# Stanford-ILIAD/PantheonRL

Measured on AMD Instinct MI355X. Metric: env-steps/sec (all agents) Overcooked-simple PPO self-play, higher is better.
Workload: dtype f32; 1 GPU; OvercookedMultiEnv-v0 layout=simple, PPO self-play (two independent PPO learners per GPU), synthetic (n_envs, n_steps, obs_dim) rollouts; n_envs=1024, n_steps=128, obs_dim=62, features=62, n_logits=6, batch_size=32768, n_epochs=10, agents_per_gpu=2, parallelism=2 agent(s) per gpu x1 gpu(s) = 2 learners (single process), launch_mode=graph, gemm_mode=2, action_masks=none, rollout=scripted, rollout_requested=scripted

## Files before the change

### pantheonrl_amd/csrc/ph_policy.hip

```cpp
#include <cstring>
#include <initializer_list>
#include "ph_rowtail.h"
#include "ph_liar_group.h"
#include "ph_pool.h"

namespace ph {


template <int R, int LP, bool VALU>
__device__ __forceinline__ void policy_fwd_body(const FwdArgs& a) {
  extern __shared__ __attribute__((aligned(16))) float smem[];
  constexpr int NT = R * 4;
  const NetDims& nd = a.nd;
  constexpr int Lp = LP, LDO = LP + 1;
  float* bufA = smem;
  float* bufB = bufA + R * LDH;
  float* w1s = bufB + R * LDH;
  float* w2s = w1s + HID * LDH;
  float* wos = w2s + HID * LDH;
  float* outs = wos + HID * LDO;
  float* b1s = outs + R * LDO;
  float* b2s = b1s + HID;
  float* bos = b2s + HID;
  int* rowphys = (int*)(bos + 64);

  const int tid = threadIdx.x;
  const int wave = tid >> 6, lane = tid & 63, li = lane & 31, lh = lane >> 5;
  const int mt = wave >> 1, nt = wave & 1;
  const int net = blockIdx.y;
  const int row0 = blockIdx.x * R;
  const ph_layout& lay = nd.lay;
  const float* W1 = a.params + (net == 0 ? lay.pi_W1 : lay.vf_W1);
  const float* B1 = a.params + (net == 0 ? lay.pi_b1 : lay.vf_b1);
  const float* W2 = a.params + (net == 0 ? lay.pi_W2 : lay.vf_W2);
  const float* B2 = a.params + (net == 0 ? lay.pi_b2 : lay.vf_b2);

  PH_STAMP(a.prof, 0);
  if (tid < R) rowphys[tid] = (row0 + tid < a.n) ? row0 + tid : -1;
  WStage<NT> w2r, w1r;
  WoStage<NT> wor;
  XStage<R, NT> xr;
  w2r.issue(W2, 0, HID);
  w1r.issue(W1, 0, nd.F);
  if (net == 0) wor.issue(a.params + lay.act_W, nd.L, Lp);
  float bias1 = 0.f, bias2 = 0.f, bias3 = 0.f;
  if (tid < HID) {
    bias1 = B1[tid];
    bias2 = B2[tid];
    bias3 = (net == 0) ? ((tid < nd.L) ? a.params[lay.act_b + tid] : 0.f) : a.params[lay.val_W + tid];
  }
  PH_STAMP(a.prof, 8);
  __syncthreads();
  PH_STAMP(a.prof, 9);
  xr.issue(rowphys, a.obs, nd, 0);
  w2r.commit(w2s);
  PH_STAMP(a.prof, 10);
  w1r.commit(w1s);
  if (net == 0) wor.commit(wos, Lp, LDO);
  if (tid < HID) {
    b1s[tid] = bias1;
    b2s[tid] = bias2;
    bos[tid] = bias3;
  }
  PH_STAMP(a.prof, 11);
  xr.commit(bufA, rowphys, a.obs, nd, 0);
  __syncthreads();
  PH_STAMP(a.prof, 1);

  f32x16 acc = {0};
  for (int c = 0; c < nd.nchunk; ++c) {
    if (c > 0) {
      __syncthreads();
      w1r.issue(W1, c * HID, nd.F);
      xr.issue(rowphys, a.obs, nd, c);
      w1r.commit(w1s);
      xr.commit(bufA, rowphys, a.obs, nd, c);
      __syncthreads();
    }
    PH_STAMP(a.prof, 2);
    acc = tile_mma<false, false, VALU>(bufA, LDH, w1s, LDH, mt * 32, nt * 32, 0, HID, acc);
  }
  PH_STAMP(a.prof, 3);
#pragma unroll
  for (int r = 0; r < 16; ++r) {
    const int row = mt * 32 + drow(r, lh), col = nt * 32 + li;
    bufB[row * LDH + col] = fast_tanh(acc[r] + b1s[col]);
  }
  __syncthreads();
  PH_STAMP(a.prof, 4);

  f32x16 acc2 = {0};
  acc2 = tile_mma<false, false, VALU>(bufB, LDH, w2s, LDH, mt * 32, nt * 32, 0, HID, acc2);
#pragma unroll
  for (int r = 0; r < 16; ++r) {
    const int row = mt * 32 + drow(r, lh), col = nt * 32 + li;
    bufA[row * LDH + col] = fast_tanh(acc2[r] + b2s[col]);
  }
  __syncthreads();
  PH_STAMP(a.prof, 5);

  if (net == 1) {
    if (tid < R && rowphys[tid] >= 0) {
      float v = 0.f;
      for (int j = 0; j < HID; ++j) v = __builtin_fmaf(bufA[tid * LDH + j], bos[j], v);
      value_row_tail(a, row0 + tid, v + a.params[lay.val_b]);
    }
    copy_obs_rows(a, row0, (a.n - row0 < R) ? a.n - row0 : R, nd.D);
    PH_STAMP(a.prof, 7);
    return;
  }

  {
    const int ntn = Lp >> 5;
    if (wave < (R >> 5) * ntn) {
      const int hm = wave / ntn, hn = wave - hm * ntn;
      f32x16 acc3 = {0};
      acc3 = tile_mma<false, false, VALU>(bufA, LDH, wos, LDO, hm * 32, hn * 32, 0, HID, acc3);
#pragma unroll
      for (int r = 0; r < 16; ++r) {
        const int row = hm * 32 + drow(r, lh), col = hn * 32 + li;
        outs[row * LDO + col] = acc3[r] + bos[col];
      }
    }
  }
  __syncthreads();
  PH_STAMP(a.prof, 6);

  if (tid < R && rowphys[tid] >= 0) general_row_tail(a, nd, row0 + tid, outs + tid * LDO, fwd_counter(a));
  PH_STAMP(a.prof, 7);
}


__device__ __forceinline__ void lds_only_barrier() { asm volatile("s_waitcnt lgkmcnt(0)\n\ts_barrier" ::: "memory"); }
__device__ __forceinline__ void vm_drain() { __builtin_amdgcn_s_waitcnt(0x0F70); }

template <int CTRL>
__device__ __forceinline__ float dpp_quad_f(float v) {
  return __builtin_bit_cast(float, __builtin_amdgcn_update_dpp(0, __builtin_bit_cast(int, v), CTRL, 0xF, 0xF, true));
}
__device__ __forceinline__ float quad_sum_f(float v) {
  v += dpp_quad_f<0xB1>(v);
  v += dpp_quad_f<0x4E>(v);
  return v;
}

template <bool KEEP_JOINT>
__device__ __forceinline__ void fwd_args_pin_lean(FwdArgs& a) {
  a.mask = nullptr;
  a.uniforms = nullptr;
  a.given_actions = nullptr;
  a.deterministic = 0;
  a.act_f32 = nullptr;
  a.entropy = nullptr;
  a.logits = nullptr;
#ifndef PH_LEAN_PROF
  a.prof = nullptr;
#endif
  a.pos_env = nullptr;
  a.rec_mask = nullptr;
  if constexpr (!KEEP_JOINT) {
    a.joint = nullptr;
    a.joint_ll = nullptr;
  }
  a.env_mask = nullptr;
  a.host_done = nullptr;
  __builtin_assume(a.rb_obs != nullptr);
  __builtin_assume(a.rb_act != nullptr);
  __builtin_assume(a.rb_rew != nullptr);
  __builtin_assume(a.rb_es != nullptr);
  __builtin_assume(a.rb_val != nullptr);
  __builtin_assume(a.rb_logp != nullptr);
  __builtin_assume(a.es_in != nullptr);
}
bool fwd_args_lean(const FwdArgs& a, bool joint_ok = false) {
  static int enabled = -1;
  if (enabled < 0) {
    const char* e = getenv("PH_ROLLOUT_LEAN");
    enabled = (e && e[0] == '0') ? 0 : 1;
  }
#ifdef PH_LEAN_PROF
  constexpr bool lean_prof = true;
#else
  constexpr bool lean_prof = false;
#endif
  return enabled && !a.mask && !a.uniforms && !a.given_actions && !a.deterministic && !a.act_f32 && !a.entropy && !a.logits && (lean_prof || !a.prof) &&
         !a.pos_env && !a.rec_mask && (joint_ok || (!a.joint && !a.joint_ll)) && !a.env_mask && !a.host_done && a.rb_obs && a.rb_act && a.rb_rew &&
         a.rb_es && a.rb_val && a.rb_logp && a.es_in;
}

constexpr int ZS_FLOATS = 4 * 16 * 8;

template <bool VALU, int LEAN = 0>
__device__ __forceinline__ void policy_fwd16_body(const FwdArgs& a0, const ph_p2p* px = nullptr, int px_t = 0, int px_a_local = 0,
                                                  int agent = 0, const ScriptedSteps* sc = nullptr, int px_persistent = 0) {
  extern __shared__ __attribute__((aligned(16))) float smem[];
  constexpr int R = 16, NT = 256;
  const NetDims& nd = a0.nd;
  FwdArgs a = a0;
  if constexpr (LEAN == 1) fwd_args_pin_lean<false>(a);
  if constexpr (LEAN == 2) fwd_args_pin_lean<true>(a);
#ifdef PH_LEAN_PROF
  long long* const prof0 = a0.prof;
#else
  long long* const prof0 = LEAN ? nullptr : a0.prof;
#endif
  float* xs = smem;
  float* hs = xs + R * LDH;
  float* zs = hs + R * LDH;
  int* rowphys = (int*)(zs + ZS_FLOATS);
  float* upre = (float*)(rowphys + 16);
  unsigned long long** pxll = (unsigned long long**)(upre + 32);

  const int tid = threadIdx.x;
  const int wave = tid >> 6, lane = tid & 63, c = lane & 15, g = lane >> 4;
  const int net = blockIdx.y;
  const int row0 = blockIdx.x * R;
  const ph_layout& lay = nd.lay;
  const float* W1 = a.params + (net == 0 ? lay.pi_W1 : lay.vf_W1);
  const float* B1 = a.params + (net == 0 ? lay.pi_b1 : lay.vf_b1);
  const float* W2 = a.params + (net == 0 ? lay.pi_W2 : lay.vf_W2);
  const float* B2 = a.params + (net == 0 ? lay.pi_b2 : lay.vf_b2);
  const int nk = nd.L;

  PH_STAMP(a.prof, 0);
  if (tid < R) rowphys[tid] = (row0 + tid < a.n) ? row0 + tid : -1;
  constexpr bool PXH = LEAN != 0;
  const int pxw_h = (PXH && px) ? px->world : 0, pxc_h = (PXH && px) ? px->count : 0, pxr_h = (PXH && px) ? px->rank : 0;
  const int pxT_h = (PXH && px) ? px->T : 1, pxslots_h = (PXH && px) ? px->ll_slots : 1;
  unsigned long long* const ll_self_h = (PXH && px) ? px->ll[pxr_h] : nullptr;
  if (PXH && px && tid < pxw_h && tid < PH_MAX_RANKS) pxll[tid] = px->ll[tid];
#define pxw (PXH ? pxw_h : px->world)
#define pxc (PXH ? pxc_h : px->count)
#define pxr (PXH ? pxr_h : px->rank)
#define pxT (PXH ? pxT_h : px->T)
#define pxslots (PXH ? pxslots_h : px->ll_slots)
#define ll_self (PXH ? ll_self_h : px->ll[px->rank])
#define PXLL(p) (PXH ? pxll[p] : px->ll[p])
  float bw1[16], bw2[16], bwh[4];
  const int col = 16 * wave + c;
#pragma unroll
  for (int s = 0; s < 16; ++s) {
    const int k = g + 4 * s;
    bw1[s] = (k < nd.F) ? W1[k * HID + col] : 0.f;
    bw2[s] = W2[k * HID + col];
  }
#pragma unroll
  for (int s = 0; s < 4; ++s) {
    const int k = g + 4 * (4 * wave + s);
    bwh[s] = 0.f;
    if (net == 0) {
      if (c < nk) bwh[s] = a.params[lay.act_W + k * nk + c];
    } else if (c == 0) {
      bwh[s] = a.params[lay.val_W + k];
    }
  }
  const float bias1 = B1[col], bias2 = B2[col];
  float hbias = 0.f;
  if (wave == 0) {
    if (net == 0) hbias = (c < nk) ? a.params[lay.act_b + c] : 0.f;
    else hbias = (c == 0) ? a.params[lay.val_b] : 0.f;
  }
  XStage<R, NT> xr;
  lds_only_barrier();
  if (sc) a.obs = sc->obs_seq;
  xr.issue(rowphys, a.obs, nd, 0);
  xr.commit(xs, rowphys, a.obs, nd, 0);
  vm_drain();
  lds_only_barrier();
  PH_STAMP(a.prof, 1);

  const int n_steps = sc ? sc->n_steps : 1;
  unsigned long long epoch_hi = 0ull;
  if (sc) {
    epoch_hi = a0.epoch ? (unsigned long long)(*a0.epoch) << 32 : 0ull;
    a.epoch = nullptr;
    a.counter = a0.counter + epoch_hi;
  }
  const unsigned long long px_epoch = (px && px_persistent) ? *px->epoch : 0ull;
  const bool draw_ahead = sc && net == 0 && !a.uniforms && !a.deterministic && !a.given_actions;
  auto draw_uniforms = [&](int t1) {
    if (lane < R && row0 + lane < a0.n)
      upre[(t1 & 1) * R + lane] = philox_uniform(a0.seed, a0.counter + (unsigned long long)t1 + epoch_hi, (uint32_t)(row0 + lane), 0u);
  };
  if (draw_ahead && wave == 1) draw_uniforms(0);

  auto product = [&](const float* A, const float (&bw)[16]) -> f32x4 {
    f32x4 e = {0.f, 0.f, 0.f, 0.f}, o = {0.f, 0.f, 0.f, 0.f};
    const float* ap = A + c * LDH + g;
    float av[16];
#pragma unroll
    for (int s = 0; s < 16; ++s) av[s] = ap[4 * s];
    __builtin_amdgcn_sched_barrier(0);
#pragma unroll
    for (int s = 0; s < 16; s += 2) {
      e = mma16<VALU>(av[s], bw[s], e, lane);
      o = mma16<VALU>(av[s + 1], bw[s + 1], o, lane);
    }
    return e + o;
  };

  for (int t = 0; t < n_steps; ++t) {
  long long* const pstep = (sc && t == 8) ? prof0 : nullptr;
  PH_STAMP(pstep, 8);
  if (t > 0) {
    const size_t row = (size_t)t * a0.n;
    a.obs = sc->obs_seq + row * nd.D;
    a.counter = a0.counter + (unsigned long long)t + epoch_hi;
    a.rb_obs = a0.rb_obs + row * nd.D;
    a.rb_act = a0.rb_act + row * nd.A;
    a.rb_rew = a0.rb_rew + row;
    a.rb_es = a0.rb_es + row;
    a.rb_val = a0.rb_val + row;
    a.rb_logp = a0.rb_logp + row;
    a.es_in = sc->done_seq + (row - a0.n);
    a.pending_reward = sc->rew_seq + (row - a0.n);
    a.prev_rew = a0.rb_rew + (row - a0.n);
    if constexpr (!LEAN) {
      a.mask = (sc->mask_seq && sc->mask_policy) ? sc->mask_seq + row * nd.L : nullptr;
      a.env_mask = (sc->mask_seq && sc->mask_env) ? sc->mask_seq + row * nd.L : nullptr;
    }
    if (px_persistent && a0.joint) {
      a.joint = a0.joint;
      a.joint_ll = ll_self + (size_t)p2p_persistent_slot(px_epoch, pxT, t - 1) * pxw * pxc;
      a.ll_t = t - 1;
    }
    a.prof = nullptr;
    xr.issue(rowphys, a.obs, nd, 0);
    xr.commit(xs, rowphys, a.obs, nd, 0);
    vm_drain();
    lds_only_barrier();
  }
  PH_STAMP(pstep, 9);

  const bool pre_ok = net == 1 && wave == 0 && lane < R && row0 + lane < a.n && !a.pos_env && a.rb_val;
  ValuePre vpre = {0.f, 0.f, 0.f, 0ull, 0ull, 0u, 0, 0};
  if (pre_ok) vpre = value_row_preload(a, row0 + lane);
  const bool copy_from_regs = net == 1 && a.rb_obs && !a.pos_env && nd.obs_kind == PH_SPACE_BOX;
  {
    const f32x4 z1 = product(xs, bw1);
#pragma unroll
    for (int r = 0; r < 4; ++r) hs[(4 * g + r) * LDH + col] = fast_tanh(z1[r] + bias1);
  }
  lds_only_barrier();
  PH_STAMP(a.prof, 3);
  PH_STAMP(pstep, 10);
  {
    const f32x4 z2 = product(hs, bw2);
#pragma unroll
    for (int r = 0; r < 4; ++r) xs[(4 * g + r) * LDH + col] = fast_tanh(z2[r] + bias2);
  }
  lds_only_barrier();
  PH_STAMP(a.prof, 5);
  PH_STAMP(pstep, 11);

  {
    if (wave == 0 && pre_ok) value_row_preload_words(a, row0 + lane, vpre);
    const float* ap = xs + c * LDH + g + 16 * wave;
    float av[4];
#pragma unroll
    for (int j = 0; j < 4; ++j) av[j] = ap[4 * j];
    f32x4 e = {0.f, 0.f, 0.f, 0.f}, o = {0.f, 0.f, 0.f, 0.f};
    e = mma16<VALU>(av[0], bwh[0], e, lane);
    o = mma16<VALU>(av[1], bwh[1], o, lane);
    e = mma16<VALU>(av[2], bwh[2], e, lane);
    o = mma16<VALU>(av[3], bwh[3], o, lane);
    const f32x4 zh = e + o;
    if (c < 8) {
#pragma unroll
      for (int r = 0; r < 4; ++r) zs[(wave * R + 4 * g + r) * 8 + c] = zh[r] + hbias;
    }
  }
  lds_only_barrier();
  PH_STAMP(pstep, 12);
  if (wave == 0) {
    PH_STAMP(pstep, 13);
    const int r = lane, grow = row0 + lane;
    if (r < R && grow < a.n) {
      float z[8];
      {
        float4 q[4][2];
#pragma unroll
        for (int w = 0; w < 4; ++w) {
          q[w][0] = *reinterpret_cast<const float4*>(zs + (w * R + r) * 8);
          q[w][1] = *reinterpret_cast<const float4*>(zs + (w * R + r) * 8 + 4);
        }
#pragma unroll
        for (int h = 0; h < 2; ++h) {
          z[4 * h + 0] = (q[0][h].x + q[1][h].x) + (q[2][h].x + q[3][h].x);
          z[4 * h + 1] = (q[0][h].y + q[1][h].y) + (q[2][h].y + q[3][h].y);
          z[4 * h + 2] = (q[0][h].z + q[1][h].z) + (q[2][h].z + q[3][h].z);
          z[4 * h + 3] = (q[0][h].w + q[1][h].w) + (q[2][h].w + q[3][h].w);
        }
      }
      if (net == 0) {
        const float* up = draw_ahead ? upre + (t & 1) * R + r : nullptr;
        const uint64_t ctr = fwd_counter(a);
        int act;
        switch (nk) {
          case 1: act = discrete8_row_tail<1>(a, nd, grow, z, ctr, up, pstep); break;
          case 2: act = discrete8_row_tail<2>(a, nd, grow, z, ctr, up, pstep); break;
          case 3: act = discrete8_row_tail<3>(a, nd, grow, z, ctr, up, pstep); break;
          case 4: act = discrete8_row_tail<4>(a, nd, grow, z, ctr, up, pstep); break;
          case 5: act = discrete8_row_tail<5>(a, nd, grow, z, ctr, up, pstep); break;
          case 6: act = discrete8_row_tail<6>(a, nd, grow, z, ctr, up, pstep); break;
          case 7: act = discrete8_row_tail<7>(a, nd, grow, z, ctr, up, pstep); break;
          default: act = discrete8_row_tail<8>(a, nd, grow, z, ctr, up, pstep); break;
        }
        if (px) {
          const int pt = px_t + t;
          const int slot = px_persistent ? p2p_persistent_slot(px_epoch, pxT, pt) : pt % pxslots;
          const size_t off = (size_t)slot * pxw * pxc + (size_t)(pxr * px_a_local + agent) * a.n + grow;
          const unsigned long long w =
              ((unsigned long long)p2p_stamp32(px_persistent ? px_epoch : *px->epoch, pxT, pt) << 32) | (unsigned long long)(unsigned)act;
          for (int p = 0; p < pxw; ++p)
            __hip_atomic_store(PXLL(p) + off, w, __ATOMIC_RELAXED, __HIP_MEMORY_SCOPE_SYSTEM);
        }
      } else {
        value_row_tail(a, grow, z[0], pre_ok, vpre);
        if (sc && t == n_steps - 1) {
          float add = sc->rew_seq[(size_t)t * a0.n + grow];
          if (px_persistent && a0.joint) {
            FwdArgs b = a;
            b.joint_ll = ll_self + (size_t)p2p_persistent_slot(px_epoch, pxT, t) * pxw * pxc;
            b.ll_t = t;
            int p = *a0.partner_seat;
            p = p < 0 ? 0 : (p >= a0.n_seats ? a0.n_seats - 1 : p);
            const int mine = ll_read(b, b.joint_ll + (size_t)a0.seat * a0.n + grow);
            const int theirs = ll_read(b, b.joint_ll + (size_t)p * a0.n + grow);
            add += joint_reward(mine, theirs, a0.bonus, a0.reward_rule);
          }
          a.rb_rew[grow] += add;
        }
      }
    }
  }
  PH_STAMP(pstep, 14);
  if (draw_ahead && wave == 1 && t + 1 < n_steps) draw_uniforms(t + 1);
  if (copy_from_regs) {
    const int kk = tid & 63;
#pragma unroll
    for (int i = 0; i < XStage<R, NT>::ITERS; ++i) {
      const int rr = (tid + NT * i) >> 6;
      if (kk < nd.D && row0 + rr < a.n) a.rb_obs[(size_t)(row0 + rr) * nd.D + kk] = xr.v[i];
    }
  } else if (net == 1) {
    copy_obs_rows(a, row0, (a.n - row0 < R) ? a.n - row0 : R, nd.D);
  }
  PH_STAMP(a.prof, 7);
  PH_STAMP(pstep, 15);
  }
}

#undef pxw
#undef pxc
#undef pxr
#undef pxT
#undef pxslots
#undef ll_self
#undef PXLL

template <bool VALU, bool LEAN = false>
__global__ __launch_bounds__(256) void policy_fwd16_kernel(FwdArgs a) {
  policy_fwd16_body<VALU, LEAN ? 1 : 0>(a);
  if constexpr (!LEAN) {
    if (a.host_done) {
      __threadfence_system();
      __syncthreads();
      if (threadIdx.x == 0) __hip_atomic_store(a.host_done + blockIdx.y, a.host_seq, __ATOMIC_RELEASE, __HIP_MEMORY_SCOPE_SYSTEM);
    }
  }
}
template <bool VALU, bool LEAN>
__global__ __launch_bounds__(256) void policy_fwd16_rollout_kernel(FwdArgs a, ScriptedSteps sc) {
  policy_fwd16_body<VALU, LEAN ? 1 : 0>(a, nullptr, 0, 0, 0, &sc);
}
template <bool LEAN>
__global__ __launch_bounds__(256) void policy_fwd16_multi_kernel(FwdMulti m) {
  policy_fwd16_body<false, LEAN ? 2 : 0>(m.a[blockIdx.z], m.px.x, m.px.t, m.px.a_local, blockIdx.z);
}
template <bool LEAN>
__global__ __launch_bounds__(256, 3) void policy_fwd16_exchange_rollout_kernel(FwdMulti m, ScriptedMulti sm) {
  policy_fwd16_body<false, LEAN ? 2 : 0>(m.a[blockIdx.z], m.px.x, 0, m.px.a_local, blockIdx.z, &sm.sc[blockIdx.z], 1);
}

static size_t fwd16_lds_bytes() { return sizeof(float) * (size_t)(2 * 16 * LDH + ZS_FLOATS + 16 + 32) + sizeof(void*) * PH_MAX_RANKS; }

bool fwd16_eligible(const NetDims& nd, int n) {
  static int enabled = -1;
  if (enabled < 0) {
    const char* e = getenv("PH_FWD16");
    enabled = (e && e[0] == '0') ? 0 : 1;
  }
  return enabled && !nd.gauss && nd.nchunk == 1 && nd.A == 1 && nd.L <= 8 && n < 16384;
}

template <bool VALU>
static hipError_t launch_fwd16_variant(const FwdArgs& a, hipStream_t s) {
  const size_t lds = fwd16_lds_bytes();
  const bool general = VALU || !fwd_args_lean(a);
  const void* fn = general ? (const void*)policy_fwd16_kernel<VALU> : (const void*)policy_fwd16_kernel<false, true>;
  if (const hipError_t e = allow_dynamic_lds(fn, lds); e != hipSuccess) return e;
  if (general) hipLaunchKernelGGL((policy_fwd16_kernel<VALU>), dim3((a.n + 15) / 16, 2), dim3(256), lds, s, a);
  else hipLaunchKernelGGL((policy_fwd16_kernel<false, true>), dim3((a.n + 15) / 16, 2), dim3(256), lds, s, a);
  return hipGetLastError();
}

static size_t rollout_lds_bytes(int nwg_total) {
  const int cu = device_cu_count();
  return (cu > 0 && 2 * nwg_total <= cu) ? (size_t)81 * 1024 + 512 : fwd16_lds_bytes();
}
hipError_t launch_policy_fwd16_rollout(const FwdArgs& a, const ScriptedSteps& sc, int gemm_mode, hipStream_t s) {
  dim3 grid((a.n + 15) / 16, 2), block(256);
  const size_t lds = rollout_lds_bytes((int)(grid.x * grid.y));
  const int variant = gemm_mode == 1 ? 1 : ((fwd_args_lean(a) && !sc.mask_seq) ? 2 : 0);
  const void* fn = variant == 1 ? (const void*)policy_fwd16_rollout_kernel<true, false>
                                : (variant == 2 ? (const void*)policy_fwd16_rollout_kernel<false, true> : (const void*)policy_fwd16_rollout_kernel<false, false>);
  if (const hipError_t e = allow_dynamic_lds(fn, lds); e != hipSuccess) return e;
  if (variant == 1) hipLaunchKernelGGL((policy_fwd16_rollout_kernel<true, false>), grid, block, lds, s, a, sc);
  else if (variant == 2) hipLaunchKernelGGL((policy_fwd16_rollout_kernel<false, true>), grid, block, lds, s, a, sc);
  else hipLaunchKernelGGL((policy_fwd16_rollout_kernel<false, false>), grid, block, lds, s, a, sc);
  return hipGetLastError();
}

hipError_t exchange_rollout_blocks_per_cu(int* blocks_out) {
  const size_t lds = fwd16_lds_bytes();
  int api = 0;
  hipError_t e = hipOccupancyMaxActiveBlocksPerMultiprocessor(&api, (const void*)policy_fwd16_exchange_rollout_kernel<false>, 256, lds);
  if (e != hipSuccess) return e;
  const int by_lds = (int)((size_t)160 * 1024 / lds);
  int blocks = api < 8 ? api : 8;
  if (blocks > by_lds) blocks = by_lds;
  else if (blocks < by_lds && blocks > 1) blocks -= 1;
  *blocks_out = blocks < 1 ? 1 : blocks;
  return hipSuccess;
}

hipError_t launch_policy_fwd16_exchange_rollout(const FwdMulti& m, const ScriptedMulti& sm, int n_agents, hipStream_t s) {
  bool lean = true;
  for (int i = 0; i < n_agents; ++i) lean = lean && fwd_args_lean(m.a[i], true) && !sm.sc[i].mask_seq;
  const dim3 grid((m.a[0].n + 15) / 16, 2, n_agents);
  if (lean) hipLaunchKernelGGL(policy_fwd16_exchange_rollout_kernel<true>, grid, dim3(256), fwd16_lds_bytes(), s, m, sm);
  else hipLaunchKernelGGL(policy_fwd16_exchange_rollout_kernel<false>, grid, dim3(256), fwd16_lds_bytes(), s, m, sm);
  return hipGetLastError();
}

template <int CTRL>
__device__ __forceinline__ float dpp_f(float v) {
  return __builtin_bit_cast(float, __builtin_amdgcn_update_dpp(0, __builtin_bit_cast(int, v), CTRL, 0xF, 0xF, true));
}
template <bool MAX>
__device__ __forceinline__ float seg_scan32(float v, int k, int lo) {
  const int kr = k & 15;
#define PH_SCAN_STEP(D, CTRL)                                   \
  {                                                             \
    const float o = dpp_f<CTRL>(v);                             \
    const bool ok = kr >= (D) && k - (D) >= lo;                 \
    v = ok ? (MAX ? fmaxf(v, o) : v + o) : v;                   \
  }
  PH_SCAN_STEP(1, 0x111)
  PH_SCAN_STEP(2, 0x112)
  PH_SCAN_STEP(4, 0x114)
  PH_SCAN_STEP(8, 0x118)
#undef PH_SCAN_STEP
  const float o = dpp_f<0x142>(v);
  const bool ok = k >= 16 && lo <= 15;
  return ok ? (MAX ? fmaxf(v, o) : v + o) : v;
}
__device__ __forceinline__ float sum32_upper(float v) {
  v += dpp_f<0xB1>(v);
  v += dpp_f<0x4E>(v);
  v += dpp_f<0x124>(v);
  v += dpp_f<0x128>(v);
  return v + dpp_f<0x142>(v);
}
__device__ __forceinline__ bool head_draws(const FwdArgs& a) { return !a.given_actions && !a.deterministic && !a.uniforms; }
__device__ __forceinline__ float head_draw32(const FwdArgs& a, int g, bool row_ok, int comp, uint64_t ctr) {
  return (row_ok && comp >= 0) ? philox_uniform(a.seed, ctr, (uint32_t)g, (uint32_t)comp) : 0.f;
}
__device__ __forceinline__ void head_tail32(const FwdArgs& a, const NetDims& nd, int g, bool row_ok, long long ridx, float z,
                                            int k, int lo, int last, int comp, float u_drawn) {
  const bool own = row_ok && comp >= 0;
  const int nk = last - lo + 1;
  if (own && a.mask) z = z - 30.0f * (1.0f - (float)(a.mask[(size_t)g * nd.L + k] != 0));
  if (own && a.logits) a.logits[(size_t)g * nd.L + k] = z;
  const float M = __shfl(seg_scan32<true>(z, k, lo), last, 32);
  const float e = fast_exp(z - M);
  const float s = seg_scan32<false>(e, k, lo);
  const float S = __shfl(s, last, 32);
  const float lse = M + fast_log(S), inv = __builtin_amdgcn_rcpf(S);
  const int half = (threadIdx.x >> 5) & 1;
  int act = 0;
  if (a.given_actions) {
    act = own ? (int)a.given_actions[(size_t)g * nd.A + comp] : 0;
    act = act < 0 ? 0 : (act >= nk ? nk - 1 : act);
  } else if (a.deterministic) {
    const unsigned long long b = __ballot(z == M);
    const unsigned bits = ((unsigned)(b >> (32 * half)) >> lo) & (nk >= 32 ? 0xffffffffu : ((1u << nk) - 1u));
    act = bits ? __ffs(bits) - 1 : 0;
  } else {
    float u = 0.f;
    if (own) u = a.uniforms ? a.uniforms[(size_t)g * nd.A + comp] : u_drawn;
    const unsigned long long b = __ballot(own && k < last && u >= s * inv);
    const unsigned bits = ((unsigned)(b >> (32 * half)) >> lo) & (nk >= 32 ? 0xffffffffu : ((1u << nk) - 1u));
    act = __popc(bits);
  }
  const float zact = __shfl(z, lo + act, 32);
  const float lp = z - lse;
  const float ent = sum32_upper(own ? -(e * inv) * lp : 0.f);
  const float logp = sum32_upper((own && k == lo) ? zact - lse : 0.f);
  if (!row_ok) return;
  if (comp >= 0 && k == lo) {
    if (a.act_i32) a.act_i32[(size_t)g * nd.A + comp] = act;
    if (a.act_f32) a.act_f32[(size_t)g * nd.A + comp] = (float)act;
    if (a.rb_act && ridx >= 0) a.rb_act[(size_t)ridx * nd.A + comp] = (float)act;
  }
  if (k == 16) {
    if (a.logp) a.logp[g] = logp;
    if (a.entropy) a.entropy[g] = ent;
    if (a.rb_logp && ridx >= 0) a.rb_logp[ridx] = logp;
  }
}

__device__ float ph_zero_row[HID];
constexpr int RES_LDO = 33;
constexpr int RES_NET_FLOATS = HID * LDH + HID * RES_LDO + HID + HID + 32;
struct ResidentNet {
  float* w2s;
  float* wos;
  float* b1s;
  float* b2s;
  float* hbs;
};
__device__ __forceinline__ ResidentNet resident_net_at(float* base) {
  ResidentNet r;
  r.w2s = base;
  r.wos = r.w2s + HID * LDH;
  r.b1s = r.wos + HID * RES_LDO;
  r.b2s = r.b1s + HID;
  r.hbs = r.b2s + HID;
  return r;
}
constexpr int RES_SCRATCH_FLOATS = 2 * 16 * LDH + 16 * 33 + 2 * 16 * 64 + 40 + 96 + 2 * 16 + 8;

template <bool MAP>
__device__ __forceinline__ int fwd16h_row(const int* map, int row, int row0, int n_end) {
  if constexpr (MAP) return map[row < n_end ? row : row0];
  else return row;
}
template <bool VALU, bool FUSED = false, bool RES = false, bool MAP = false>
__device__ __forceinline__ void policy_fwd16h_body(const FwdArgs& a, int row0_in = 0, int net_in = 0, int tid_in = 0,
                                                   float* smem_in = nullptr, int row_end_in = 0,
                                                   const ResidentNet resv = ResidentNet{nullptr, nullptr, nullptr, nullptr, nullptr},
                                                   const int* ooff = nullptr, const int* map = nullptr, int map_n = 0) {
  const ResidentNet* const res = &resv;
  extern __shared__ __attribute__((aligned(16))) float smem_dyn[];
  float* smem = FUSED ? smem_in : smem_dyn;
  constexpr int R = 16, NT = 256, LDO = 33, FS = 64;
  constexpr int LDW = RES ? RES_LDO : LDH;
  const NetDims& nd = a.nd;
  float* xs = smem;
  float* hs = xs + R * LDH;
  float* w2s = RES ? res->w2s : hs + R * LDH;
  float* wos = RES ? res->wos : w2s + HID * LDH;
  float* outs = RES ? hs + R * LDH : wos + HID * LDH;
  float* b2s = RES ? res->b2s : outs + R * LDO;
  float* hbs = RES ? res->hbs : b2s + HID;
  const float** feat = (const float**)(RES ? outs + R * LDO : hbs + 32);
  int* aoff = (int*)(feat + R * FS);
  int* seg = aoff + 40;
  long long* ridxs = (long long*)(seg + 96);

  const int tid = FUSED ? tid_in : (int)threadIdx.x;
  const int wave = tid >> 6, lane = tid & 63, c = lane & 15, g = lane >> 4;
  const int net = FUSED ? net_in : (int)blockIdx.y;
  const int row0 = (FUSED || MAP) ? row0_in : (int)blockIdx.x * R;
  const int n_end = MAP ? map_n : (FUSED ? row_end_in : a.n);
  const ph_layout& lay = nd.lay;
  const float* W1 = a.params + (net == 0 ? lay.pi_W1 : lay.vf_W1);
  const float* B1 = a.params + (net == 0 ? lay.pi_b1 : lay.vf_b1);
  const float* W2 = a.params + (net == 0 ? lay.pi_W2 : lay.vf_W2);
  const float* B2 = a.params + (net == 0 ? lay.pi_b2 : lay.vf_b2);
  const int D = nd.D;

  PH_STAMP(a.prof, 0);
  const float* fv[R * FS / NT];
  {
    const int* off = RES ? ooff : nd.obs_off;
    int lo[R * FS / NT], hi[R * FS / NT];
    float xo[R * FS / NT];
#pragma unroll
    for (int i = 0; i < R * FS / NT; ++i) {
      const int r = 4 * wave + i, comp = lane, row = row0 + r;
      const bool ok = comp < D && row < n_end;
      const int cs = ok ? comp : 0, rs = ok ? row : row0;
      lo[i] = off[cs];
      hi[i] = off[cs + 1];
      xo[i] = a.obs[(size_t)fwd16h_row<MAP>(map, rs, row0, n_end) * D + cs];
    }
#pragma unroll
    for (int i = 0; i < R * FS / NT; ++i) {
      const int r = 4 * wave + i, comp = lane, row = row0 + r;
      const int nn = hi[i] - lo[i];
      int x = (int)xo[i];
      x = x < 0 ? 0 : (x >= nn ? nn - 1 : x);
      fv[i] = (comp < D && row < n_end) ? W1 + (size_t)(lo[i] + x) * HID : ph_zero_row;
    }
  }
  long long ridxv = -1;
  if (net == 0 && tid < R && row0 + tid < n_end && (a.rb_act || a.rb_logp)) ridxv = rb_row(a, fwd16h_row<MAP>(map, row0 + tid, row0, n_end));
  WStage<NT> w2r;
  const int gr = tid >> 4, gl = tid & 15;
  float b1v[4];
  float bias2 = 0.f, hb = 0.f, hv[8];
  int aoffv = 0;
  if constexpr (!RES) {
    w2r.issue(W2, 0, HID, tid);
#pragma unroll
    for (int i = 0; i < 4; ++i) b1v[i] = B1[4 * gl + i];
    if (tid < HID) bias2 = B2[tid];
    if (net == 0) {
      if (tid <= nd.A) aoffv = nd.act_off[tid];
#pragma unroll
      for (int i = 0; i < 8; ++i) {
        const int e = tid + NT * i, j = e >> 5, k = e & 31;
        hv[i] = (k < nd.L) ? a.params[lay.act_W + j * nd.L + k] : 0.f;
      }
      if (tid < 32) hb = (tid < nd.L) ? a.params[lay.act_b + tid] : 0.f;
    } else {
      hv[0] = (tid < HID) ? a.params[lay.val_W + tid] : 0.f;
      if (tid == 0) hb = a.params[lay.val_b];
    }
  } else {
#pragma unroll
    for (int i = 0; i < 4; ++i) b1v[i] = res->b1s[4 * gl + i];
  }
#pragma unroll
  for (int i = 0; i < R * FS / NT; ++i) feat[(4 * wave + i) * FS + lane] = fv[i];
  if (net == 0 && tid < R) ridxs[tid] = ridxv;
  __builtin_amdgcn_wave_barrier();
  asm volatile("s_waitcnt lgkmcnt(0)" ::: "memory");
  __builtin_amdgcn_wave_barrier();
  PH_STAMP(a.prof, 1);

  float4 acc = make_float4(0.f, 0.f, 0.f, 0.f);
  float u_tail[2] = {0.f, 0.f};
  const float* const* fr = feat + gr * FS;
// ... 857 lines not shown
```

Measured before the change: 115.7 million agent-steps/s.

## Prefetch next-step observation rows with buffer loads during current step compute

In the scripted multi-step rollout kernel, waves 1-3 now issue raw buffer loads for the next timestep's observation rows while the current step's hidden layers and head run. They commit them into shared memory afterward and copy them straight to the rollout buffer, replacing the per-step stage-in at the top of the loop. This is meant to hide global-load latency behind compute and to merge the rb_obs copy with the staging. It relies on row-index assumptions (identity row mapping, D up to 64, 16 rows) and adds extra drains and register pressure. It also changes the value tail preload flag.

```diff
diff --git a/pantheonrl_amd/csrc/ph_policy.hip b/pantheonrl_amd/csrc/ph_policy.hip
--- a/pantheonrl_amd/csrc/ph_policy.hip
+++ b/pantheonrl_amd/csrc/ph_policy.hip
@@ -133,6 +133,42 @@
 
 __device__ __forceinline__ void lds_only_barrier() { asm volatile("s_waitcnt lgkmcnt(0)\n\ts_barrier" ::: "memory"); }
 __device__ __forceinline__ void vm_drain() { __builtin_amdgcn_s_waitcnt(0x0F70); }
+
+struct RowStage3 {
+  static constexpr int ITERS = 6;
+  static constexpr unsigned NONE = 0x80000000u;
+  float v[ITERS] = {0.f, 0.f, 0.f, 0.f, 0.f, 0.f};
+  __device__ __forceinline__ static unsigned base_offset(int row0, const NetDims& nd, int tid) {
+    const int kk = tid & 63, w = (tid >> 6) - 1;
+    return (w >= 0 && kk < nd.D && kk < nd.F) ? ((unsigned)(row0 + w) * (unsigned)nd.D + (unsigned)kk) * 4u : NONE;
+  }
+  __device__ __forceinline__ static unsigned slot_offset(unsigned base, int i, int D, int tid) {
+    return (i == 5 && (tid >> 6) != 1) ? NONE : base + (unsigned)(3 * i) * (unsigned)D * 4u;
+  }
+  __device__ __forceinline__ static __amdgpu_buffer_rsrc_t block(const float* blk, int n, int D) {
+    return __builtin_amdgcn_make_buffer_rsrc(const_cast<float*>(blk), 0, n * D * 4, 0x00020000);
+  }
+  __device__ __forceinline__ void issue(const float* obs, int n, const NetDims& nd, unsigned base, int tid) {
+    const __amdgpu_buffer_rsrc_t rs = block(obs, n, nd.D);
+#pragma unroll
+    for (int i = 0; i < ITERS; ++i)
+      v[i] = __builtin_bit_cast(float, __builtin_amdgcn_raw_buffer_load_b32(rs, slot_offset(base, i, nd.D, tid), 0, 0));
+  }
+  __device__ __forceinline__ void commit(float* dst, int tid) const {
+    const int kk = tid & 63, w = (tid >> 6) - 1;
+#pragma unroll
+    for (int i = 0; i < ITERS; ++i) {
+      const int r = w + 3 * i;
+      if (r < 16) dst[r * LDH + kk] = v[i];
+    }
+  }
+  __device__ __forceinline__ void copy_out(float* rb_obs, int n, int D, unsigned base, int tid) const {
+    const __amdgpu_buffer_rsrc_t rs = block(rb_obs, n, D);
+#pragma unroll
+    for (int i = 0; i < ITERS; ++i)
+      __builtin_amdgcn_raw_buffer_store_b32(__builtin_bit_cast(unsigned, v[i]), rs, slot_offset(base, i, D, tid), 0, 0);
+  }
+};
 
 template <int CTRL>
 __device__ __forceinline__ float dpp_quad_f(float v) {
@@ -264,8 +300,14 @@
   lds_only_barrier();
   if (sc) a.obs = sc->obs_seq;
   xr.issue(rowphys, a.obs, nd, 0);
+  const bool staged = sc != nullptr && nd.obs_kind == PH_SPACE_BOX;
+  const bool copy_staged = staged && net == 1 && a.rb_obs && !a.pos_env && wave != 0;
+  const unsigned roff = RowStage3::base_offset(row0, nd, tid);
+  RowStage3 rows;
+  if (copy_staged) rows.issue(a.obs, a0.n, nd, roff, tid);
   xr.commit(xs, rowphys, a.obs, nd, 0);
   vm_drain();
+  if (copy_staged) rows.copy_out(a.rb_obs, a0.n, nd.D, roff, tid);
   lds_only_barrier();
   PH_STAMP(a.prof, 1);
 
@@ -325,12 +367,16 @@
       a.ll_t = t - 1;
     }
     a.prof = nullptr;
-    xr.issue(rowphys, a.obs, nd, 0);
-    xr.commit(xs, rowphys, a.obs, nd, 0);
-    vm_drain();
+    if (!staged) {
+      xr.issue(rowphys, a.obs, nd, 0);
+      xr.commit(xs, rowphys, a.obs, nd, 0);
+      vm_drain();
+    }
     lds_only_barrier();
   }
   PH_STAMP(pstep, 9);
+  const bool more = t + 1 < n_steps;
+  const float* const obs_next = sc ? sc->obs_seq + (size_t)(t + 1) * a0.n * nd.D : nullptr;
 
   const bool pre_ok = net == 1 && wave == 0 && lane < R && row0 + lane < a.n && !a.pos_env && a.rb_val;
   ValuePre vpre = {0.f, 0.f, 0.f, 0ull, 0ull, 0u, 0, 0};
@@ -352,6 +398,8 @@
   lds_only_barrier();
   PH_STAMP(a.prof, 5);
   PH_STAMP(pstep, 11);
+
+  if (staged && net == 1 && more && wave != 0) rows.issue(obs_next, a0.n, nd, roff, tid);
 
   {
     if (wave == 0 && pre_ok) value_row_preload_words(a, row0 + lane, vpre);
@@ -372,6 +420,13 @@
   }
   lds_only_barrier();
   PH_STAMP(pstep, 12);
+  if (sc) vm_drain();
+  if (staged && more && wave != 0) {
+    if (net == 1) {
+      rows.commit(xs, tid);
+      if (copy_staged) rows.copy_out(a0.rb_obs + (size_t)(t + 1) * a0.n * nd.D, a0.n, nd.D, roff, tid);
+    }
+  }
   if (wave == 0) {
     PH_STAMP(pstep, 13);
     const int r = lane, grow = row0 + lane;
@@ -416,7 +471,7 @@
             __hip_atomic_store(PXLL(p) + off, w, __ATOMIC_RELAXED, __HIP_MEMORY_SCOPE_SYSTEM);
         }
       } else {
-        value_row_tail(a, grow, z[0], pre_ok, vpre);
+        value_row_tail(a, grow, z[0], !a.pos_env && a.rb_val, vpre);
         if (sc && t == n_steps - 1) {
           float add = sc->rew_seq[(size_t)t * a0.n + grow];
           if (px_persistent && a0.joint) {
@@ -435,13 +490,21 @@
     }
   }
   PH_STAMP(pstep, 14);
-  if (draw_ahead && wave == 1 && t + 1 < n_steps) draw_uniforms(t + 1);
+  const bool stage_here = staged && net == 0 && more && wave != 0;
+  if (stage_here) rows.issue(obs_next, a0.n, nd, roff, tid);
+  if (draw_ahead && wave == 1 && more) draw_uniforms(t + 1);
+  if (stage_here) {
+    rows.commit(xs, tid);
+    vm_drain();
+  }
   if (copy_from_regs) {
-    const int kk = tid & 63;
-#pragma unroll
-    for (int i = 0; i < XStage<R, NT>::ITERS; ++i) {
-      const int rr = (tid + NT * i) >> 6;
-      if (kk < nd.D && row0 + rr < a.n) a.rb_obs[(size_t)(row0 + rr) * nd.D + kk] = xr.v[i];
+    if (!staged) {
+      const int kk = tid & 63;
+#pragma unroll
+      for (int i = 0; i < XStage<R, NT>::ITERS; ++i) {
+        const int rr = (tid + NT * i) >> 6;
+        if (kk < nd.D && row0 + rr < a.n) a.rb_obs[(size_t)(row0 + rr) * nd.D + kk] = xr.v[i];
+      }
     }
   } else if (net == 1) {
     copy_obs_rows(a, row0, (a.n - row0 < R) ? a.n - row0 : R, nd.D);
```

Measured after the change: 118.6 million agent-steps/s (median of 6 runs). +2.5%, better.
